# harvard-edge/multilingual_kws

Hardware: AMD Instinct MI355X
Metric: clips/sec end-to-end (log-mel + embedding fwd), batch 1024, 1s@16kHz (higher is better)
Workload: dtype f32; 1 GPU; configs[2]: batch=1024/GPU synthetic 1s@16kHz clips -> micro-frontend (int16 fixed-point, fp32 I/O) -> EfficientNet-B0 embedding forward (frozen, fp32 MFMA pointwise conv) -> [1024,1024]; clips_per_gpu=1024, samples_per_clip=16000, weights=synthetic seed 1234, parallelism=clip-sharded x1, build=47cee32cb12851f8

## Files before the change

multilingual_kws_amd/csrc/mkws_embed.hip:

```cpp
#include "mkws_common.h"
#include "mkws_embed_arch.h"

#include <algorithm>
#include <cmath>
#include <cstdlib>
#include <map>
#include <mutex>
#include <new>
#include <set>
#include <string>
#include <type_traits>
#include <vector>

#pragma clang fp contract(fast)
#include "mkws_embed_dev.h"
#include "mkws_embed_rows.h"

namespace mkws {

__device__ __forceinline__ int opaque_(int v) { asm volatile("" : "+v"(v)); return v; }
__device__ __forceinline__ float apply_act(float v, int act) {
  switch (act) {
    case ACT_SWISH: return swishf_(v);
    case ACT_RELU: return v > 0.0f ? v : 0.0f;
// ... 1014 lines not shown
  static constexpr int MTI = (G * HW + 15) / 16, MTO = (G * HoWo + 15) / 16;
  static constexpr int NW4 = KCT * NTC * 64, NS1 = NW4 + 2 * Q, NS2 = KS * KS * Q + 2 * Q;
  static constexpr int oX = 0;
  static constexpr int oS1 = oX + KCT * MTI * 256;
  static constexpr int oS2 = oS1 + NS1 * 4;
  static constexpr int oE = oS2 + NS2 * 4;
  static constexpr int oD = oE + (G * HW + 1) * LDE;
  static constexpr int oMean = oD + G * HoWo * LDD;
  static constexpr int oGate = oMean + G * CEXP;
  static constexpr int oR = oGate + G * CEXP;
  static constexpr int lds_floats = oR + G * 16;
  static_assert(NSEG * SEG == WoT, "segments tile the output row");
  static_assert(CEXP % CC == 0 && CC % 16 == 0, "chunks are whole MFMA tiles");
};

template <int KS, int S, int KCT, int HT, int WT, int CEXP, int CC, int NTP, int G, int SEG, int NTHR, int WPE, bool PAIR = false>
__global__ __launch_bounds__(NTHR, WPE) void mbconv_mid_kernel(MidArgs a) {
  using GM = MidGeom<KS, S, KCT, HT, WT, CEXP, CC, G, SEG>;
  constexpr int HW = GM::HW, HoT = GM::HoT, WoT = GM::WoT, HoWo = GM::HoWo, PT = GM::PT, PLF = GM::PLF;
  constexpr int NSEG = GM::NSEG, NC = GM::NC, Q = GM::Q, NTC = GM::NTC, LDE = GM::LDE, LDD = GM::LDD, NCH = GM::NCH, KC = GM::KC;
  constexpr int MTI = GM::MTI, MTO = GM::MTO, NW4 = GM::NW4, NS1 = GM::NS1, NS2 = GM::NS2;
  constexpr int NW = NTHR / 64;
  constexpr int SE_MAX = 10;
  constexpr int TAP_ROW_UNROLL = (KS == 5) ? 1 : KS;
  constexpr int NSL = NTHR / 16;
  constexpr int CPS = (CEXP + NSL - 1) / NSL;
  constexpr int CQ = CEXP / 4;
  constexpr int RS = NTHR / (G * CQ);
  constexpr int R1 = (NS1 + NTHR - 1) / NTHR, R2 = (NS2 + NTHR - 1) / NTHR;
  static_assert(NTHR % 64 == 0 && NTHR >= CEXP && NTHR >= 16 * G && RS >= 1, "thread roles");
  static_assert(NTHR * G <= KCT * MTI * 256 && G * RS * CEXP <= GM::oD - GM::oS1, "aliased scratch fits");
  extern __shared__ __attribute__((aligned(16))) float s_mid[];
  MKWS_WG_BEGIN();
  float* s_X = s_mid + GM::oX;
  float* s_part = s_X;
  float* s_W = s_mid + GM::oS1;
  float* s_scE = s_W + NW4 * 4;
  float* s_wd = s_mid + GM::oS2;
  float* s_scD = s_wd + KS * KS * CC;
  float* s_E = s_mid + GM::oE;
  f32x4* s_csum = reinterpret_cast<f32x4*>(s_W);
  float* s_D = s_mid + GM::oD;
  float* s_mean = s_mid + GM::oMean;
  float* s_gate = s_mid + GM::oGate;
  float* s_r = s_mid + GM::oR;
  const int tid = threadIdx.x, lane = tid & 63;
  const int wave = __builtin_amdgcn_readfirstlane(tid >> 6);
  const int g = lane >> 4, c = lane & 15;
  const int b0 = blockIdx.x * G;
  const int gvalid = (a.B - b0 < G) ? (a.B - b0) : G;
  const int rows = gvalid * HW, rows_out = gvalid * HoWo;
  const size_t row0_in = (size_t)b0 * HW, row0_out = (size_t)b0 * HoWo;
#ifdef MKWS_FRONT_TIMING
  unsigned long long* dbgp = a.dbg_t + (size_t)blockIdx.x * 8;
  unsigned long long t_p1 = 0, t_p2 = 0, t_red = 0, t_mark = 0;
  if (tid == 0) { t_mark = wall_clock64(); dbgp[0] = t_mark; }
#endif
  auto src1 = [&](int e, int chn) -> const float* {
    if (e < NW4) {
      const int l = e & 63, jn = e >> 6, j = jn / NTC, ntl = jn - j * NTC;
      return a.WpE + (((size_t)j * a.NTtotE + chn * NTC + ntl) * 64 + l) * 4;
    }
    const int q = e - NW4;
    return (q < Q ? a.scE + 4 * q : a.shE + 4 * (q - Q)) + chn * CC;
  };
  auto src2 = [&](int e, int chn) -> const float* {
    if (e < KS * KS * Q) {
      const int t = e / Q, q = e - t * Q;
      return a.Wd + (size_t)t * CEXP + chn * CC + 4 * q;
    }
    const int q = e - KS * KS * Q;
// ... 161 lines not shown
      }
    }
    if (chn + 1 < NCH) store1();
    __syncthreads();
#ifdef MKWS_FRONT_TIMING
    if (tid == 0) { const unsigned long long t = wall_clock64(); t_p2 += t - t_mark; t_mark = t; }
#endif
  }
  if (MKWS_ABLATE(16)) request_se();
  constexpr int NWP = NW / NTP;
  constexpr int MTW = (MTO + NWP - 1) / NWP;
  constexpr int PD = (KC >= 8) ? 8 : 4;
  const int ntp = wave % NTP, rlp = wave / NTP;
  const WBuf p_w(a.WpP, (unsigned)(g * 64 + c * 4));
  f32x4 wqp[PD][1];
  if (rlp < NWP) stream_mfma_prefetch<1, PD>(wqp, p_w, (size_t)NTP * 256, ntp, 1, NTP, KC);
  if (a.dbg_dw) {
    for (int i = tid; i < rows_out * CQ; i += NTHR) {
      const int r = i / CQ, q4 = (i - r * CQ) * 4;
      *reinterpret_cast<f32x4*>(a.dbg_dw + (row0_out + r) * CEXP + q4) = *reinterpret_cast<const f32x4*>(s_D + (size_t)r * LDD + q4);
    }
  }
  if (!MKWS_ABLATE(4)) {
  if (tid < G * RS * CQ) {
    const int q = tid % CQ, rs = (tid / CQ) % RS, gi = tid / (CQ * RS);
    f32x4 t = {0.f, 0.f, 0.f, 0.f};
    for (int r = rs; r < HoWo; r += RS) t += *reinterpret_cast<const f32x4*>(s_D + (size_t)(gi * HoWo + r) * LDD + 4 * q);
    s_csum[tid] = t;
  }
  __syncthreads();
  if (tid < G * CQ) {
    const int q = tid % CQ, gi = tid / CQ;
    f32x4 t = s_csum[(size_t)gi * RS * CQ + q];
#pragma unroll 4
    for (int rs = 1; rs < RS; ++rs) t += s_csum[((size_t)gi * RS + rs) * CQ + q];
    *reinterpret_cast<f32x4*>(s_mean + (size_t)gi * CEXP + 4 * q) = t * (1.0f / (float)HoWo);
  }
  __syncthreads();
  {
    const int n = tid & 15, sl = tid >> 4;
#pragma unroll
    for (int gi = 0; gi < G; ++gi) {
      float v = 0.0f;
// ... 18 lines not shown
#pragma unroll
    for (int gi = 0; gi < G; ++gi) {
      float v = be_pre;
#pragma unroll
      for (int n2 = 0; n2 < SE_MAX; ++n2) v += s_r[gi * 16 + n2] * we_pre[n2];
      const float gt = sigmoidf_(v);
      s_gate[gi * CEXP + tid] = gt;
      if (a.dbg_gate && gi < gvalid) a.dbg_gate[(size_t)(b0 + gi) * CEXP + tid] = gt;
    }
  }
  __syncthreads();
  }
#ifdef MKWS_FRONT_TIMING
  if (tid == 0) { const unsigned long long t = wall_clock64(); t_red += t - t_mark; t_mark = t; }
#endif
  if (rlp < NWP && !MKWS_ABLATE(8)) {
    constexpr int MT_LO = MTO / NWP;
    const int my_tiles = (MTO - rlp + NWP - 1) / NWP;
    auto run = [&](auto mt_tag) {
      constexpr int MT = decltype(mt_tag)::value;
      const float* erow[MT];
      const float* grow[MT];
#pragma unroll
      for (int m = 0; m < MT; ++m) {
        int r = (rlp + NWP * m) * 16 + c;
        if (r >= G * HoWo) r = G * HoWo - 1;
        erow[m] = s_D + (size_t)r * LDD + 4 * g;
        grow[m] = s_gate + (size_t)(r / HoWo) * CEXP + 4 * g;
      }
      struct EG { f32x4 e, g; };
      auto xload = [&](int j, int m) { return EG{*reinterpret_cast<const f32x4*>(erow[m] + 16 * j), *reinterpret_cast<const f32x4*>(grow[m] + 16 * j)}; };
// ... 13 lines not shown
            if (a.residual) y += *reinterpret_cast<const f32x4*>(a.X + (row0_in + r) * a.Cin + n);
            *reinterpret_cast<f32x4*>(a.Y + (row0_out + r) * a.Cout + n) = y;
          }
        }
      }
    };
    if constexpr (MT_LO >= 1 && MT_LO < MTW) {
      if (my_tiles >= MTW) run(std::integral_constant<int, MTW>{});
      else run(std::integral_constant<int, MT_LO>{});
    } else {
      run(std::integral_constant<int, MTW>{});
    }
  }
#ifdef MKWS_FRONT_TIMING
  __syncthreads();
  if (tid == 0) { const unsigned long long t = wall_clock64(); dbgp[1] = t_p1; dbgp[2] = t_p2; dbgp[3] = t_red; dbgp[4] = t - t_mark; dbgp[5] = t; }
#endif
  MKWS_WG_END();
}

struct BackArgs {
  const float* D; const float* X; int Cin;
  const float* Wr; const float* br; const float* We; const float* be; int se;
  const float* WpP; const float* scP; const float* shP;
  float* Y; int Cout; int residual;
  float* dbg_gate;
  int B;
};

template <int HOWO, int CEXP, int NTP, int RS, int NTHR, int WPE>
__global__ __launch_bounds__(NTHR, WPE) void mbconv_back_kernel(BackArgs a) {
  constexpr int LDD = CEXP + 4, CQ = CEXP / 4, KC = CEXP / 16, MTO = (HOWO + 15) / 16, NW = NTHR / 64;
// ... 655 lines not shown
#ifdef MKWS_FRONT_TIMING
  __syncthreads();
  if (threadIdx.x == 0) { a.dbg_t[(size_t)blockIdx.x * 8 + 6] = wall_clock64(); a.dbg_t[(size_t)blockIdx.x * 8 + 7] = (unsigned long long)(clock64() - dbg_c0); }
#endif
}

constexpr int kChainMax = 6;
struct ChainArgs {
  const BlockArgs* tab;
  int i0, n;
  unsigned kinds;
  const float* X; float* Y;
  int B;
  int ldsU, ldsE;
  int se4;
#ifdef MKWS_FRONT_TIMING
  unsigned long long* dbg_t;
#endif
};

__device__ __forceinline__ int sgpr_(int v) { return __builtin_amdgcn_readfirstlane(v); }
template <typename T>
__device__ __forceinline__ T* sgpr_(T* p) {
  const unsigned long long v = reinterpret_cast<unsigned long long>(p);
  const unsigned lo = (unsigned)__builtin_amdgcn_readfirstlane((int)(unsigned)v), hi = (unsigned)__builtin_amdgcn_readfirstlane((int)(unsigned)(v >> 32));
  typedef __attribute__((address_space(1))) T* gptr_t;
  return (T*)reinterpret_cast<gptr_t>(((unsigned long long)hi << 32) | lo);
}
__device__ __forceinline__ BlockArgs sgpr_block_args(const BlockArgs& t) {
  BlockArgs a;
// ... 355 lines not shown
template <int MT, int NWAVES>
__global__ __launch_bounds__(NWAVES * 64) void mbconv_chain_kernel(ChainArgs ca) {
  extern __shared__ __attribute__((aligned(16))) float s_blk[];
  constexpr int NTHR = NWAVES * 64;
  constexpr int HW = 12, G = MT * 16 / HW;
  const BlockArgs* __restrict__ tab = ca.tab + ca.i0;
  const int tid = threadIdx.x, lane = tid & 63;
  const int wave = __builtin_amdgcn_readfirstlane(tid >> 6);
  const int g = lane >> 4, c = lane & 15;
#ifdef MKWS_FRONT_TIMING
  if (ca.dbg_t && threadIdx.x == 0) ca.dbg_t[(size_t)gridDim.x * kChainMax * 8 + blockIdx.x] = wall_clock64();
#endif
  f32x4 carry[MT];
#pragma unroll
  for (int m = 0; m < MT; ++m) carry[m] = (f32x4){0.f, 0.f, 0.f, 0.f};
  {
    const int Cin = sgpr_(tab[0].Cin), KCe = sgpr_(tab[0].KCe), Cexp = sgpr_(tab[0].Cexp);
    const int b0 = blockIdx.x * G;
    const int gvalid = (ca.B - b0 < G) ? (ca.B - b0) : G;
    const int rows_in = gvalid * HW;
    const size_t row0_in = (size_t)b0 * HW;
    float* s_X = s_blk;
    float* s_scE = s_blk + ca.ldsU + ca.ldsE;
    for (int jm = wave; jm < KCe * MT; jm += NWAVES) {
      const int j = jm / MT, m = jm - j * MT;
      const int r = m * 16 + c;
      f32x4 v = {0.f, 0.f, 0.f, 0.f};
      if (r < rows_in && 16 * j + 4 * g < Cin) v = *reinterpret_cast<const f32x4*>(ca.X + (row0_in + r) * Cin + 16 * j + 4 * g);
      *reinterpret_cast<f32x4*>(s_X + ((size_t)jm * 64 + lane) * 4) = v;
    }
    const float* scE = sgpr_(tab[0].scE); const float* shE = sgpr_(tab[0].shE);
// ... 1 lines not shown
    __syncthreads();
  }
  for (int i = 0; i < ca.n; ++i) {
    BlockArgs a = sgpr_block_args(tab[i]);
    const bool last = (i + 1 == ca.n);
    if (!ca.se4) a.WrQ = nullptr;
    a.X = ca.X; a.Y = ca.Y; a.B = ca.B;
    const BlockArgs* nxp = last ? tab + i : tab + i + 1;
    const unsigned kind = (ca.kinds >> (2 * i)) & 3u;
#ifdef MKWS_FRONT_TIMING
    unsigned long long* dt = ca.dbg_t ? ca.dbg_t + ((size_t)blockIdx.x * kChainMax + i) * 8 : nullptr;
    if (dt && threadIdx.x == 0) dt[7] = wall_clock64();
#else
    unsigned long long* dt = nullptr;
#endif
    if (kind == 0) chain_block<3, 1, MT, NWAVES>(a, nxp, !last, s_blk, ca.ldsU, ca.ldsE, i == 0, carry, dt);
    else if (kind == 1) chain_block<5, 1, MT, NWAVES>(a, nxp, !last, s_blk, ca.ldsU, ca.ldsE, i == 0, carry, dt);
    else chain_block<5, 2, MT, NWAVES>(a, nxp, !last, s_blk, ca.ldsU, ca.ldsE, i == 0, carry, dt);
  }
}

#ifdef MKWS_PAIR_NT_STORES
#define MKWS_XSTORE(ptr, val) __builtin_nontemporal_store((val), (ptr))
#else
#define MKWS_XSTORE(ptr, val) (*(ptr) = (val))
#endif

struct PairArgs {
  BlockArgs b;
  float* xc1;
  float* xd;
  int* flags;
  int* err_dev;
// ... 1402 lines not shown
  float* se_part = nullptr;
  float* splitk_ws = nullptr; size_t splitk_floats = 0;
  const float *stem_w = nullptr, *stem_scale = nullptr, *stem_shift = nullptr;
  float norm_mean = 0.f, norm_std = 1.f;
  bool fuse_front = true;
  int fuse_gap = 1;
  int fuse_stem = 1;
  int fuse_back = 1;
  int fuse_mid = 1;
  int fuse_gemv = 1;
  int fuse_se4 = 1;
  int fuse_walk = 1;
  int fuse_rows = 0;
  int fuse_block = 2;
  int fuse_chain = 1;
  mkws::BlockArgs* d_chain_tab = nullptr;
  int fuse_top = 1;
  int fuse_pair = 1;
  float* pair_xc1 = nullptr; float* pair_xd = nullptr; int* pair_flags = nullptr;
  int* pair_err_dev = nullptr;
  int* pair_err_host = nullptr;
  size_t pair_flag_count = 0;
  int* pair_chain_flags = nullptr;
  int pair_fault = 0;
  int pair_degraded = 0;
  int fuse_cluster = 0;
  float* cl_xc1 = nullptr; float* cl_xd = nullptr; int* cl_flags = nullptr; size_t cl_flag_count = 0;
  int fuse_cluster_chain = 0;
  int pair_mt = 2;
  int block_mt43 = 3;
// ... 478 lines not shown
}
static bool chain_link_ok(const BlockPlan& b, const BlockPlan& next) {
  if (b.spec.stride != 1) return false;
  if (b.project.NTtot > kBlockWaves) return false;
  if (next.spec.in_ch != b.spec.out_ch || next.expand.KC != b.project.NTtot) return false;
  return next.ce <= 3 * kBlockWaves * 64;
}
bool cluster_supported(const BlockPlan& b);
bool pair_supported(const BlockPlan& b);
static bool chain_member(const mkws_embed* em, const BlockPlan& b) {
  if (!(em->fuse_chain == 1 || em->fuse_chain == 2) || !em->fuse_block || !block_supported(b, em->fuse_block)) return false;
  if (!(b.H == 4 && b.W == 3)) return false;
  if (em->fuse_cluster && cluster_supported(b) && em->cl_flags) return false;
  return true;
}
int launch_chain(hipStream_t s, const mkws_embed* em, int i0, int i1, const float* X, float* Y, int B) {
  ChainArgs ca;
  const int n = i1 - i0 + 1, mt43 = em->block_mt43;
  if (!em->d_chain_tab) return fail(MKWS_ERR_UNSUPPORTED, "chain: no block table");
  ca.tab = em->d_chain_tab; ca.i0 = i0; ca.n = n; ca.kinds = 0; ca.ldsU = ca.ldsE = 0;
  ca.X = X; ca.Y = Y; ca.B = B; ca.se4 = em->fuse_se4;
  int ldsZ = 0;
  std::string names;
  for (int k = 0; k < n; ++k) {
    const BlockPlan& b = em->blocks[i0 + k];
    const int ks = b.spec.kernel, st = b.spec.stride;
    if (ks == 3 && st != 1) return fail(MKWS_ERR_UNSUPPORTED, "chain: 3x3 stride-2 block");
    ca.kinds |= (unsigned)((ks == 3 && st == 1) ? 0 : (ks == 5 && st == 1) ? 1 : 2) << (2 * k);
    const int MT = block_row_tiles(b, mt43), G = MT * 16 / (b.H * b.W);
    const BlockLds L = block_lds(b.expand.KC, b.ce, MT, G, kBlockWaves);
    ca.ldsU = std::max(ca.ldsU, L.U); ca.ldsE = std::max(ca.ldsE, L.E); ldsZ = std::max(ldsZ, L.Z);
    names += (k ? "," : "") + std::string(b.spec.name);
  }
  const size_t lds = ((size_t)ca.ldsU + ca.ldsE + ldsZ) * sizeof(float);
  if (lds > 160 * 1024) return fail(MKWS_ERR_UNSUPPORTED, "chain: LDS carve %zu bytes", lds);
  const int G = mt43 * 16 / 12;
  const dim3 grid((B + G - 1) / G);
  ProfScope ps("chain:" + names, std::string("mbconv_chain_kernel<") + std::to_string(mt43) + "," + std::to_string(kBlockWaves) + ">");
#ifdef MKWS_FRONT_TIMING
  static unsigned long long* d_ct = nullptr;
  const size_t nstamp = (size_t)grid.x * kChainMax * 8 + grid.x;
  if (!d_ct) (void)hipMalloc(&d_ct, sizeof(unsigned long long) * (4096 * kChainMax * 8 + 4096));
  ca.dbg_t = (grid.x <= 4096) ? d_ct : nullptr;
#endif
  if (mt43 == 3) {
    if (int rc_ = ensure_dynamic_lds(reinterpret_cast<const void*>(&mbconv_chain_kernel<3, kBlockWaves>), 160 * 1024)) return rc_;
    hipLaunchKernelGGL((mbconv_chain_kernel<3, kBlockWaves>), grid, dim3(kBlockWaves * 64), lds, s, ca);
  } else if (mt43 == 2) {
    if (int rc_ = ensure_dynamic_lds(reinterpret_cast<const void*>(&mbconv_chain_kernel<2, kBlockWaves>), 160 * 1024)) return rc_;
    hipLaunchKernelGGL((mbconv_chain_kernel<2, kBlockWaves>), grid, dim3(kBlockWaves * 64), lds, s, ca);
  } else {
    if (int rc_ = ensure_dynamic_lds(reinterpret_cast<const void*>(&mbconv_chain_kernel<1, kBlockWaves>), 160 * 1024)) return rc_;
    hipLaunchKernelGGL((mbconv_chain_kernel<1, kBlockWaves>), grid, dim3(kBlockWaves * 64), lds, s, ca);
  }
#ifdef MKWS_FRONT_TIMING
  if (ca.dbg_t) {
    (void)hipStreamSynchronize(s);
    std::vector<unsigned long long> h(nstamp);
    (void)hipMemcpy(h.data(), d_ct, nstamp * 8, hipMemcpyDeviceToHost);
    unsigned long long t0 = ~0ull, t1 = 0;
    for (unsigned w = 0; w < grid.x; ++w) {
      t0 = std::min(t0, h[(size_t)grid.x * kChainMax * 8 + w]);
      t1 = std::max(t1, h[((size_t)w * kChainMax + (n - 1)) * 8 + 6]);
    }
    double pro = 0;
    for (unsigned w = 0; w < grid.x; ++w) pro += (double)(h[((size_t)w * kChainMax) * 8 + 7] - h[(size_t)grid.x * kChainMax * 8 + w]);
    fprintf(stderr, "[chain-timing] %s: %u workgroups, span %.2f us, prologue %.2f us\n", names.c_str(), grid.x, (double)(t1 - t0) / 100.0, pro / grid.x / 100.0);
    for (int k = 0; k < n; ++k) {
      double ph[7] = {0, 0, 0, 0, 0, 0, 0};
      unsigned long long e_min = ~0ull, e_max = 0;
      for (unsigned w = 0; w < grid.x; ++w) {
        const unsigned long long* q = &h[((size_t)w * kChainMax + k) * 8];
        ph[0] += (double)(q[0] - q[7]);
        for (int j = 0; j < 6; ++j) ph[j + 1] += (double)(q[j + 1] - q[j]);
        e_min = std::min(e_min, q[6]); e_max = std::max(e_max, q[6]);
      }
      fprintf(stderr, "[chain-timing]   %s: args %.2f  A %.2f  B %.2f  C1 %.2f  C2 %.2f  gate %.2f  D %.2f us; end skew %.2f us\n", em->blocks[i0 + k].spec.name,
              ph[0] / grid.x / 100.0, ph[1] / grid.x / 100.0, ph[2] / grid.x / 100.0, ph[3] / grid.x / 100.0, ph[4] / grid.x / 100.0, ph[5] / grid.x / 100.0,
              ph[6] / grid.x / 100.0, (double)(e_max - e_min) / 100.0);
    }
  }
#endif
// ... 307 lines not shown
          stage, CC, G, grid.x, NTHR, lds, p1 / grid.x / 100.0, p2 / grid.x / 100.0, se / grid.x / 100.0, pj / grid.x / 100.0, tot / grid.x / 100.0, (double)(t1 - t0) / 100.0);
  MKWS_WG_TRACE_REPORT(s, stage, "mid", (size_t)grid.x);
#else
  hipLaunchKernelGGL(fn, grid, dim3(NTHR), lds, s, a);
#endif
  return MKWS_OK;
}

bool mid_enabled(const BlockPlan& b, int fuse_mid) {
  if (!fuse_mid || !mid_supported(b)) return false;
  if (fuse_mid == 2) return true;
  if (b.H == 13 && b.spec.kernel == 3) return fuse_mid == 1;
  return (b.H == 13 && b.spec.kernel == 5) || (b.H == 7 && b.spec.stride == 2);
}

int launch_mid(hipStream_t s, const char* stage, const BlockPlan& b, int one_clip, const float* X, float* Y, float* dbg_dw, float* dbg_gate, int B) {
  MidArgs a;
  a.X = X; a.Cin = b.spec.in_ch;
  a.WpE = b.expand.Wp; a.scE = b.expand.scale; a.shE = b.expand.shift; a.NTtotE = b.expand.NTtot;
  a.Wd = b.dw.Wd; a.scD = b.dw.scale; a.shD = b.dw.shift;
  a.Wr = b.se.Wr; a.br = b.se.br; a.We = b.se.We; a.be = b.se.be; a.se = b.se.se;
  a.WpP = b.project.Wp; a.scP = b.project.scale; a.shP = b.project.shift;
  a.Y = Y; a.Cout = b.spec.out_ch; a.residual = b.residual ? 1 : 0;
  a.dbg_dw = dbg_dw; a.dbg_gate = dbg_gate; a.B = B;
  const int ks = b.spec.kernel, st = b.spec.stride;
  if (b.H == 25) return launch_mid_inst<3, 2, 1, 25, 20, 96, 16, 2, 1, 1, 1024, 4>(s, stage, a);
  if (b.H == 13 && ks == 3) return launch_mid_inst<3, 1, 2, 13, 10, 144, 48, 2, 1, 5, 1024, 4, true>(s, stage, a);
  if (b.H == 13) return launch_mid_inst<5, 2, 2, 13, 10, 144, 48, 3, 1, 5, 512, 4, true>(s, stage, a);
  if (st == 1) return launch_mid_inst<5, 1, 3, 7, 5, 240, 48, 3, 1, 1, 512, 4>(s, stage, a);
  if (one_clip) return launch_mid_inst<3, 2, 3, 7, 5, 240, 48, 5, 1, 3, 512, 4, true>(s, stage, a);
  return launch_mid_inst<3, 2, 3, 7, 5, 240, 48, 5, 2, 3, 512, 4, true>(s, stage, a);
}

int rows_variant(const BlockPlan& b) {
  if (!b.has_expand || b.se.se > 10 || b.spec.stride != 1 || !b.residual) return -1;
  const int ks = b.spec.kernel, ci = b.spec.in_ch, co = b.spec.out_ch;
  if (b.H == 13 && b.W == 10 && ks == 3 && ci == 24 && co == 24 && b.ce == 144 && b.project.NTtot == 2) return kRows2b;
  if (b.H == 7 && b.W == 5 && ks == 5 && ci == 40 && co == 40 && b.ce == 240 && b.project.NTtot == 3) return kRows3b;
  return -1;
// ... 117 lines not shown
#ifdef MKWS_FRONT_TIMING
    wg_phase_report("block1a: prologue / stem / depthwise + next stage / SE / projection", (size_t)(B < device_cu_count() ? B : device_cu_count()), 5);
#endif
  } else {
    const long pix = (long)B * 500;
    int grid = (int)((pix + 31) / 32);
    if (grid > 8192) grid = 8192;
    ProfScope ps("stem", "stem_kernel");
    hipLaunchKernelGGL(stem_kernel, dim3(grid), dim3(256), 0, s, d_spec, em->stem_w, em->stem_scale, em->stem_shift,
                       em->norm_mean, em->norm_std, em->bufA, B);
    if (hit("stem", em->bufA, (size_t)B * 500 * kStemCh)) return MKWS_OK;
  }
  float* cur = em->bufA;
  float* nxt = em->bufB;
  bool top_done = false;
  for (int i = 0; i < kNumBlocks; ++i) {
    const BlockPlan& b = em->blocks[i];
    const std::string p = std::string("block") + b.spec.name;
    const int Min = B * b.H * b.W, Mout = B * b.Ho * b.Wo;
    if (i == 0 && fused_1a) {
      if (hit(p, nxt, (size_t)Mout * b.spec.out_ch)) return MKWS_OK;
      float* t = cur; cur = nxt; nxt = t;
      continue;
    }
    const bool want_expand_tap = stop && (p + "_expand") == stop;
    if (em->fuse_rows && rows_variant(b) >= 0 && !want_expand_tap) {
      const bool tap_dw = stop && (p + "_dw") == stop, tap_gate = stop && (p + "_gate") == stop;
      if (int rc = launch_rows(s, p.c_str(), b, em->fuse_rows == 2, cur, nxt, tap_dw ? em->bufD : nullptr, tap_gate ? em->gate : nullptr, B)) return rc;
      if (hit(p + "_dw", em->bufD, (size_t)Mout * b.ce)) return MKWS_OK;
      if (hit(p + "_gate", em->gate, (size_t)B * b.ce)) return MKWS_OK;
      if (hit(p, nxt, (size_t)Mout * b.spec.out_ch)) return MKWS_OK;
      float* t = cur; cur = nxt; nxt = t;
      continue;
    }
    if (mid_enabled(b, em->fuse_mid) && !want_expand_tap) {
      const bool tap_dw = stop && (p + "_dw") == stop, tap_gate = stop && (p + "_gate") == stop;
      if (int rc = launch_mid(s, p.c_str(), b, em->block_mt43 == 1, cur, nxt, tap_dw ? em->bufD : nullptr, tap_gate ? em->gate : nullptr, B)) return rc;
      if (hit(p + "_dw", em->bufD, (size_t)Mout * b.ce)) return MKWS_OK;
      if (hit(p + "_gate", em->gate, (size_t)B * b.ce)) return MKWS_OK;
      if (hit(p, nxt, (size_t)Mout * b.spec.out_ch)) return MKWS_OK;
      float* t = cur; cur = nxt; nxt = t;
      continue;
    }
    {
      auto inner_tap = [&](int j) {
        if (!stop) return false;
        const std::string q = std::string("block") + em->blocks[j].spec.name;
        return (q + "_expand") == stop || (q + "_dw") == stop || (q + "_gate") == stop;
      };
      if (chain_member(em, b) && !inner_tap(i)) {
        int e = i;
        while (e + 1 < kNumBlocks && e + 1 - i < kChainMax && !(stop && (std::string("block") + em->blocks[e].spec.name) == stop) &&
               chain_member(em, em->blocks[e + 1]) && chain_link_ok(em->blocks[e], em->blocks[e + 1]) && !inner_tap(e + 1)) ++e;
        const BlockPlan& bl = em->blocks[e];
        if (int rc = launch_chain(s, em, i, e, cur, nxt, B)) return rc;
        if (hit(std::string("block") + bl.spec.name, nxt, (size_t)B * bl.Ho * bl.Wo * bl.spec.out_ch)) return MKWS_OK;
        float* t = cur; cur = nxt; nxt = t;
        i = e;
        continue;
      }
      if (pair_chain_member(em, b) && !inner_tap(i)) {
        int e = i;
        while (e + 1 < kNumBlocks && e + 1 - i < kPairChainMax && !(stop && (std::string("block") + em->blocks[e].spec.name) == stop) &&
               pair_chain_member(em, em->blocks[e + 1]) && pair_chain_link_ok(em->blocks[e], em->blocks[e + 1]) && !inner_tap(e + 1)) ++e;
        const BlockPlan& bl = em->blocks[e];
        const bool with_top = em->fuse_top && em->fuse_gap && (!stop || strcmp(stop, "gap") == 0 || strncmp(stop, "dense", 5) == 0) && e == kNumBlocks - 1 && em->topH * em->topW == 4;
        if (int rc = launch_pair_chain(s, em, i, e, cur, nxt, B, with_top)) return rc;
        top_done = with_top;
        if (hit(std::string("block") + bl.spec.name, nxt, (size_t)B * bl.Ho * bl.Wo * bl.spec.out_ch)) return MKWS_OK;
        float* t = cur; cur = nxt; nxt = t;
        i = e;
        continue;
      }
    }
    if (B == 1 && em->fuse_block && em->fuse_cluster_chain && cluster_supported(b) && !stop) {
// ... 350 lines not shown
  return MKWS_OK;
}

int mkws_embed_set_option(mkws_embed* em, const char* name, int value) {
  if (!em || !name) return fail(MKWS_ERR_INVALID_ARG, "NULL argument");
  if (strcmp(name, "fuse_front") == 0) { em->fuse_front = value != 0; return MKWS_OK; }
  if (strcmp(name, "fuse_block") == 0) { em->fuse_block = value; return MKWS_OK; }
  if (strcmp(name, "fuse_mid") == 0) { em->fuse_mid = value; return MKWS_OK; }
  if (strcmp(name, "fuse_rows") == 0) { em->fuse_rows = value; return MKWS_OK; }
  if (strcmp(name, "fuse_walk") == 0) { em->fuse_walk = value; return MKWS_OK; }
  if (strcmp(name, "fuse_se4") == 0) { em->fuse_se4 = value ? 1 : 0; return MKWS_OK; }
  if (strcmp(name, "fuse_gemv") == 0) { em->fuse_gemv = value; return MKWS_OK; }
  if (strcmp(name, "fuse_back") == 0) { em->fuse_back = value; return MKWS_OK; }
  if (strcmp(name, "fuse_pair") == 0) { em->fuse_pair = value; return MKWS_OK; }
  if (strcmp(name, "fuse_chain") == 0) { em->fuse_chain = value; return MKWS_OK; }
  if (strcmp(name, "fuse_top") == 0) { em->fuse_top = value; return MKWS_OK; }
  if (strcmp(name, "fuse_cluster") == 0) {
    if (value && !em->cl_flags) return fail(MKWS_ERR_UNSUPPORTED, "fuse_cluster needs a handle of at most 64 clips (max_batch = %d)", em->max_batch);
    em->fuse_cluster = value; return MKWS_OK;
  }
  if (strcmp(name, "fuse_cluster_chain") == 0) {
    if (value && (em->max_batch != 1 || !em->cl_flags)) return fail(MKWS_ERR_UNSUPPORTED, "fuse_cluster_chain is the plan of one-clip handles (max_batch = %d)", em->max_batch);
    em->fuse_cluster_chain = value; return MKWS_OK;
  }
  if (strcmp(name, "fuse_stem") == 0) { em->fuse_stem = value; return MKWS_OK; }
  if (strcmp(name, "big_tiles") == 0) {
    if (value) { em->pair_mt = 2; em->block_mt43 = 3; } else { em->pair_mt = pair_row_tiles(em->plan_batch); em->block_mt43 = block43_row_tiles(em->plan_batch); }
    return MKWS_OK;
  }
  if (strcmp(name, "plan_batch") == 0) {
// ... 20 lines not shown
  return fail(MKWS_ERR_INVALID_ARG, "unknown option '%s'", name);
}

int mkws_embed_get_option(const mkws_embed* em, const char* name) {
  if (!em || !name) return fail(MKWS_ERR_INVALID_ARG, "NULL argument");
  if (strcmp(name, "fuse_front") == 0) return em->fuse_front ? 1 : 0;
  if (strcmp(name, "fuse_block") == 0) return em->fuse_block;
  if (strcmp(name, "fuse_mid") == 0) return em->fuse_mid;
  if (strcmp(name, "fuse_rows") == 0) return em->fuse_rows;
  if (strcmp(name, "fuse_walk") == 0) return em->fuse_walk;
  if (strcmp(name, "fuse_se4") == 0) return em->fuse_se4;
  if (strcmp(name, "fuse_gemv") == 0) return em->fuse_gemv;
  if (strcmp(name, "fuse_back") == 0) return em->fuse_back;
  if (strcmp(name, "fuse_pair") == 0) return em->fuse_pair;
  if (strcmp(name, "fuse_chain") == 0) return em->fuse_chain;
  if (strcmp(name, "fuse_top") == 0) return em->fuse_top;
  if (strcmp(name, "fuse_cluster") == 0) return em->fuse_cluster;
  if (strcmp(name, "fuse_cluster_chain") == 0) return em->fuse_cluster_chain;
  if (strcmp(name, "fuse_stem") == 0) return em->fuse_stem;
  if (strcmp(name, "fuse_gap") == 0) return em->fuse_gap;
  if (strcmp(name, "block_tiles") == 0) return em->block_mt43;
  if (strcmp(name, "pair_degraded") == 0) return em->pair_degraded;
  if (strcmp(name, "guard_floats") == 0) return (int)em->guard;
  if (strcmp(name, "guard_bands") == 0) return (int)em->guard_spans.size();
  if (strcmp(name, "guard_violations") == 0) return guard_violations(em);
  if (strcmp(name, "exchange_error") == 0) return em->pair_err_host ? *reinterpret_cast<volatile int*>(em->pair_err_host) : 0;
  if (strcmp(name, "max_batch") == 0) return em->max_batch;
  if (strcmp(name, "plan_batch") == 0) return em->plan_batch;
  return fail(MKWS_ERR_INVALID_ARG, "unknown option '%s'", name);
}
// ... 50 lines not shown
```

Baseline: 1.092 million clips/s.

## Fuse block 4a mid kernel into the following chain kernel as a prologue

Refactors the mid kernel body into a device function and calls it as a prologue inside the chain kernel for block 4a (stride-2, 240 expand). The projected output stays in LDS as MFMA fragments and is handed to the first chain block as its carry, so the 4a output never goes through global memory and one kernel launch is dropped. A new wave dealing gives the last row tile's projection to the extra waves. The cost is that the chain kernel now needs the larger LDS carve of the two stages, which may lower occupancy, and the scale and shift loads have to be staged around the prologue.

```diff
diff --git a/multilingual_kws_amd/csrc/mkws_embed.hip b/multilingual_kws_amd/csrc/mkws_embed.hip
--- a/multilingual_kws_amd/csrc/mkws_embed.hip
+++ b/multilingual_kws_amd/csrc/mkws_embed.hip
@@ -1052,8 +1052,8 @@
   static_assert(CEXP % CC == 0 && CC % 16 == 0, "chunks are whole MFMA tiles");
 };
 
-template <int KS, int S, int KCT, int HT, int WT, int CEXP, int CC, int NTP, int G, int SEG, int NTHR, int WPE, bool PAIR = false>
-__global__ __launch_bounds__(NTHR, WPE) void mbconv_mid_kernel(MidArgs a) {
+template <int KS, int S, int KCT, int HT, int WT, int CEXP, int CC, int NTP, int G, int SEG, int NTHR, bool PAIR, int RSF, bool LINK>
+__device__ __forceinline__ void mid_body(const MidArgs& a, float* s_mid) {
   using GM = MidGeom<KS, S, KCT, HT, WT, CEXP, CC, G, SEG>;
   constexpr int HW = GM::HW, HoT = GM::HoT, WoT = GM::WoT, HoWo = GM::HoWo, PT = GM::PT, PLF = GM::PLF;
   constexpr int NSEG = GM::NSEG, NC = GM::NC, Q = GM::Q, NTC = GM::NTC, LDE = GM::LDE, LDD = GM::LDD, NCH = GM::NCH, KC = GM::KC;
@@ -1064,12 +1064,10 @@
   constexpr int NSL = NTHR / 16;
   constexpr int CPS = (CEXP + NSL - 1) / NSL;
   constexpr int CQ = CEXP / 4;
-  constexpr int RS = NTHR / (G * CQ);
+  constexpr int RS = RSF ? RSF : NTHR / (G * CQ);
   constexpr int R1 = (NS1 + NTHR - 1) / NTHR, R2 = (NS2 + NTHR - 1) / NTHR;
-  static_assert(NTHR % 64 == 0 && NTHR >= CEXP && NTHR >= 16 * G && RS >= 1, "thread roles");
+  static_assert(NTHR % 64 == 0 && NTHR >= CEXP && NTHR >= 16 * G && NTHR >= G * CQ && RS >= 1, "thread roles");
   static_assert(NTHR * G <= KCT * MTI * 256 && G * RS * CEXP <= GM::oD - GM::oS1, "aliased scratch fits");
-  extern __shared__ __attribute__((aligned(16))) float s_mid[];
-  MKWS_WG_BEGIN();
   float* s_X = s_mid + GM::oX;
   float* s_part = s_X;
   float* s_W = s_mid + GM::oS1;
@@ -1090,9 +1088,9 @@
   const int rows = gvalid * HW, rows_out = gvalid * HoWo;
   const size_t row0_in = (size_t)b0 * HW, row0_out = (size_t)b0 * HoWo;
 #ifdef MKWS_FRONT_TIMING
-  unsigned long long* dbgp = a.dbg_t + (size_t)blockIdx.x * 8;
+  unsigned long long* dbgp = a.dbg_t ? a.dbg_t + (size_t)blockIdx.x * 8 : nullptr;
   unsigned long long t_p1 = 0, t_p2 = 0, t_red = 0, t_mark = 0;
-  if (tid == 0) { t_mark = wall_clock64(); dbgp[0] = t_mark; }
+  if (tid == 0 && dbgp) { t_mark = wall_clock64(); dbgp[0] = t_mark; }
 #endif
   auto src1 = [&](int e, int chn) -> const float* {
     if (e < NW4) {
@@ -1284,7 +1282,14 @@
   const int ntp = wave % NTP, rlp = wave / NTP;
   const WBuf p_w(a.WpP, (unsigned)(g * 64 + c * 4));
   f32x4 wqp[PD][1];
-  if (rlp < NWP) stream_mfma_prefetch<1, PD>(wqp, p_w, (size_t)NTP * 256, ntp, 1, NTP, KC);
+  const bool lrow = LINK && wave >= NTP;
+  const int lt0 = 2 * (wave - NTP);
+  f32x4 wql[PD][2];
+  if (LINK) {
+    static_assert(!LINK || (MTO >= 2 && MTO * 16 == G * HoWo && NTP <= 2 * (NW - NTP) && NTP <= NW), "link dealing");
+    if (!lrow) stream_mfma_prefetch<1, PD>(wqp, p_w, (size_t)NTP * 256, wave, 1, NTP, KC);
+    else stream_mfma_prefetch<2, PD>(wql, p_w, (size_t)NTP * 256, lt0, 1, NTP, KC);
+  } else if (rlp < NWP) stream_mfma_prefetch<1, PD>(wqp, p_w, (size_t)NTP * 256, ntp, 1, NTP, KC);
   if (a.dbg_dw) {
     for (int i = tid; i < rows_out * CQ; i += NTHR) {
       const int r = i / CQ, q4 = (i - r * CQ) * 4;
@@ -1292,11 +1297,11 @@
     }
   }
   if (!MKWS_ABLATE(4)) {
-  if (tid < G * RS * CQ) {
-    const int q = tid % CQ, rs = (tid / CQ) % RS, gi = tid / (CQ * RS);
+  for (int it = tid; it < G * RS * CQ; it += NTHR) {
+    const int q = it % CQ, rs = (it / CQ) % RS, gi = it / (CQ * RS);
     f32x4 t = {0.f, 0.f, 0.f, 0.f};
     for (int r = rs; r < HoWo; r += RS) t += *reinterpret_cast<const f32x4*>(s_D + (size_t)(gi * HoWo + r) * LDD + 4 * q);
-    s_csum[tid] = t;
+    s_csum[it] = t;
   }
   __syncthreads();
   if (tid < G * CQ) {
@@ -1345,7 +1350,49 @@
 #ifdef MKWS_FRONT_TIMING
   if (tid == 0) { const unsigned long long t = wall_clock64(); t_red += t - t_mark; t_mark = t; }
 #endif
-  if (rlp < NWP && !MKWS_ABLATE(8)) {
+  if constexpr (LINK) {
+   if (!MKWS_ABLATE(8)) {
+    struct EG { f32x4 e, g; };
+    auto xmake = [](const EG& v) { return v.e * v.g; };
+    auto rows_of = [&](int rt, const float*& er, const float*& gr) {
+      const int r = rt * 16 + c;
+      er = s_D + (size_t)r * LDD + 4 * g;
+      gr = s_gate + (size_t)(r / HoWo) * CEXP + 4 * g;
+    };
+    auto fin = [&](const f32x4& acc, int t, int rt) {
+      const int n = t * 16 + 4 * g, r = rt * 16 + c;
+      f32x4 y = {0.f, 0.f, 0.f, 0.f};
+      if (r < rows_out) {
+        y = acc * *reinterpret_cast<const f32x4*>(a.scP + n) + *reinterpret_cast<const f32x4*>(a.shP + n);
+        if (a.residual) y += *reinterpret_cast<const f32x4*>(a.X + (row0_in + r) * a.Cin + n);
+      }
+      *reinterpret_cast<f32x4*>(s_mid + ((size_t)(t * MTO + rt) * 64 + lane) * 4) = y;
+    };
+    if (!lrow) {
+      constexpr int MT = MTO - 1;
+      const float* erow[MT];
+      const float* grow[MT];
+#pragma unroll
+      for (int m = 0; m < MT; ++m) rows_of(m, erow[m], grow[m]);
+      auto xload = [&](int j, int m) { return EG{*reinterpret_cast<const f32x4*>(erow[m] + 16 * j), *reinterpret_cast<const f32x4*>(grow[m] + 16 * j)}; };
+      f32x4 acc[1][MT];
+#pragma unroll
+      for (int m = 0; m < MT; ++m) acc[0][m] = (f32x4){0.f, 0.f, 0.f, 0.f};
+      stream_mfma<1, PD, MT, true>(acc, wqp, p_w, (size_t)NTP * 256, wave, 1, NTP, KC, xload, xmake);
+#pragma unroll
+      for (int m = 0; m < MT; ++m) fin(acc[0][m], wave, m);
+    } else {
+      const float* er; const float* gr;
+      rows_of(MTO - 1, er, gr);
+      auto xload = [&](int j, int) { return EG{*reinterpret_cast<const f32x4*>(er + 16 * j), *reinterpret_cast<const f32x4*>(gr + 16 * j)}; };
+      f32x4 acc[2][1] = {{{0.f, 0.f, 0.f, 0.f}}, {{0.f, 0.f, 0.f, 0.f}}};
+      stream_mfma<2, PD, 1, true>(acc, wql, p_w, (size_t)NTP * 256, lt0, 1, NTP, KC, xload, xmake);
+#pragma unroll
+      for (int q = 0; q < 2; ++q)
+        if (lt0 + q < NTP) fin(acc[q][0], lt0 + q, MTO - 1);
+    }
+   }
+  } else if (rlp < NWP && !MKWS_ABLATE(8)) {
     constexpr int MT_LO = MTO / NWP;
     const int my_tiles = (MTO - rlp + NWP - 1) / NWP;
     auto run = [&](auto mt_tag) {
@@ -1389,8 +1436,15 @@
   }
 #ifdef MKWS_FRONT_TIMING
   __syncthreads();
-  if (tid == 0) { const unsigned long long t = wall_clock64(); dbgp[1] = t_p1; dbgp[2] = t_p2; dbgp[3] = t_red; dbgp[4] = t - t_mark; dbgp[5] = t; }
-#endif
+  if (tid == 0 && dbgp) { const unsigned long long t = wall_clock64(); dbgp[1] = t_p1; dbgp[2] = t_p2; dbgp[3] = t_red; dbgp[4] = t - t_mark; dbgp[5] = t; }
+#endif
+}
+
+template <int KS, int S, int KCT, int HT, int WT, int CEXP, int CC, int NTP, int G, int SEG, int NTHR, int WPE, bool PAIR = false>
+__global__ __launch_bounds__(NTHR, WPE) void mbconv_mid_kernel(MidArgs a) {
+  extern __shared__ __attribute__((aligned(16))) float s_mid[];
+  MKWS_WG_BEGIN();
+  mid_body<KS, S, KCT, HT, WT, CEXP, CC, NTP, G, SEG, NTHR, PAIR, 0, false>(a, s_mid);
   MKWS_WG_END();
 }
 
@@ -2076,6 +2130,8 @@
   int B;
   int ldsU, ldsE;
   int se4;
+  int link4a;
+  MidArgs a4;
 #ifdef MKWS_FRONT_TIMING
   unsigned long long* dbg_t;
 #endif
@@ -2461,7 +2517,45 @@
   f32x4 carry[MT];
 #pragma unroll
   for (int m = 0; m < MT; ++m) carry[m] = (f32x4){0.f, 0.f, 0.f, 0.f};
-  {
+  bool link = false;
+  if constexpr (MT == 3) link = ca.link4a != 0;
+  if constexpr (MT == 3) {
+    if (link) {
+      constexpr int NCST = 3;
+      const int Cexp = sgpr_(tab[0].Cexp);
+      float nsc[NCST], nsh[NCST];
+      {
+        const float* scE = sgpr_(tab[0].scE); const float* shE = sgpr_(tab[0].shE);
+#pragma unroll
+        for (int k = 0; k < NCST; ++k) {
+          const int i = tid + k * NTHR;
+          if (i < Cexp) { nsc[k] = scE[i]; nsh[k] = shE[i]; }
+        }
+      }
+      mid_body<3, 2, 3, 7, 5, 240, 48, 5, 4, 3, NTHR, true, 4, true>(ca.a4, s_blk);
+      __syncthreads();
+      const int NTp = sgpr_(tab[0].NTp);
+      const bool rowsplit = (NTp == NWAVES / 2 + 1) && (MT <= NWAVES / 2 - 1);
+      auto frag = [&](int t, int m) { return *reinterpret_cast<const f32x4*>(s_blk + ((size_t)(t * MT + m) * 64 + lane) * 4); };
+      if (rowsplit) {
+        if (wave < NWAVES / 2) {
+#pragma unroll
+          for (int m = 0; m < MT; ++m) carry[m] = frag(wave, m);
+        } else if (wave < NWAVES / 2 + MT) carry[0] = frag(NTp - 1, wave - NWAVES / 2);
+      } else if (wave < NTp) {
+#pragma unroll
+        for (int m = 0; m < MT; ++m) carry[m] = frag(wave, m);
+      }
+      float* s_scE = s_blk + ca.ldsU + ca.ldsE;
+#pragma unroll
+      for (int k = 0; k < NCST; ++k) {
+        const int i = tid + k * NTHR;
+        if (i < Cexp) { s_scE[i] = nsc[k]; s_scE[Cexp + i] = nsh[k]; }
+      }
+      __syncthreads();
+    }
+  }
+  if (!link) {
     const int Cin = sgpr_(tab[0].Cin), KCe = sgpr_(tab[0].KCe), Cexp = sgpr_(tab[0].Cexp);
     const int b0 = blockIdx.x * G;
     const int gvalid = (ca.B - b0 < G) ? (ca.B - b0) : G;
@@ -2493,9 +2587,10 @@
 #else
     unsigned long long* dt = nullptr;
 #endif
-    if (kind == 0) chain_block<3, 1, MT, NWAVES>(a, nxp, !last, s_blk, ca.ldsU, ca.ldsE, i == 0, carry, dt);
-    else if (kind == 1) chain_block<5, 1, MT, NWAVES>(a, nxp, !last, s_blk, ca.ldsU, ca.ldsE, i == 0, carry, dt);
-    else chain_block<5, 2, MT, NWAVES>(a, nxp, !last, s_blk, ca.ldsU, ca.ldsE, i == 0, carry, dt);
+    const bool first = i == 0 && !link;
+    if (kind == 0) chain_block<3, 1, MT, NWAVES>(a, nxp, !last, s_blk, ca.ldsU, ca.ldsE, first, carry, dt);
+    else if (kind == 1) chain_block<5, 1, MT, NWAVES>(a, nxp, !last, s_blk, ca.ldsU, ca.ldsE, first, carry, dt);
+    else chain_block<5, 2, MT, NWAVES>(a, nxp, !last, s_blk, ca.ldsU, ca.ldsE, first, carry, dt);
   }
 }
 
@@ -3928,6 +4023,7 @@
   int fuse_rows = 0;
   int fuse_block = 2;
   int fuse_chain = 1;
+  int fuse_chain_4a = 1;
   mkws::BlockArgs* d_chain_tab = nullptr;
   int fuse_top = 1;
   int fuse_pair = 1;
@@ -4436,14 +4532,29 @@
   if (em->fuse_cluster && cluster_supported(b) && em->cl_flags) return false;
   return true;
 }
-int launch_chain(hipStream_t s, const mkws_embed* em, int i0, int i1, const float* X, float* Y, int B) {
+using Link4aGeom = MidGeom<3, 2, 3, 7, 5, 240, 48, 4, 3>;
+void fill_mid_args(MidArgs& a, const BlockPlan& b, const float* X, float* Y, float* dbg_dw, float* dbg_gate, int B);
+bool mid_enabled(const BlockPlan& b, int fuse_mid);
+static bool chain_link4a_ok(const mkws_embed* em, const BlockPlan& b, const BlockPlan& first) {
+  return em->fuse_chain_4a && em->block_mt43 == 3 && mid_enabled(b, em->fuse_mid) && b.H == 7 && b.W == 5 && b.spec.stride == 2 && b.spec.kernel == 3 &&
+         b.ce == 240 && b.spec.in_ch == 40 && b.spec.out_ch == 80 && b.project.NTtot == 5 && first.spec.stride == 1 && first.spec.in_ch == 80 &&
+         first.expand.KC == 5 && first.ce <= 3 * kBlockWaves * 64 && (size_t)Link4aGeom::lds_floats * sizeof(float) <= 160 * 1024;
+}
+int launch_chain(hipStream_t s, const mkws_embed* em, int i0, int i1, const float* X, float* Y, int B, const BlockPlan* link4a = nullptr) {
   ChainArgs ca;
   const int n = i1 - i0 + 1, mt43 = em->block_mt43;
   if (!em->d_chain_tab) return fail(MKWS_ERR_UNSUPPORTED, "chain: no block table");
   ca.tab = em->d_chain_tab; ca.i0 = i0; ca.n = n; ca.kinds = 0; ca.ldsU = ca.ldsE = 0;
   ca.X = X; ca.Y = Y; ca.B = B; ca.se4 = em->fuse_se4;
+  ca.link4a = 0; ca.a4 = MidArgs{};
   int ldsZ = 0;
   std::string names;
+  if (link4a) {
+    if (mt43 != 3 || !chain_link4a_ok(em, *link4a, em->blocks[i0])) return fail(MKWS_ERR_UNSUPPORTED, "chain: 4a link on this plan");
+    ca.link4a = 1;
+    fill_mid_args(ca.a4, *link4a, X, nullptr, nullptr, nullptr, B);
+    names = std::string(link4a->spec.name) + ",";
+  }
   for (int k = 0; k < n; ++k) {
     const BlockPlan& b = em->blocks[i0 + k];
     const int ks = b.spec.kernel, st = b.spec.stride;
@@ -4454,7 +4565,8 @@
     ca.ldsU = std::max(ca.ldsU, L.U); ca.ldsE = std::max(ca.ldsE, L.E); ldsZ = std::max(ldsZ, L.Z);
     names += (k ? "," : "") + std::string(b.spec.name);
   }
-  const size_t lds = ((size_t)ca.ldsU + ca.ldsE + ldsZ) * sizeof(float);
+  size_t lds = ((size_t)ca.ldsU + ca.ldsE + ldsZ) * sizeof(float);
+  if (link4a) lds = std::max(lds, (size_t)Link4aGeom::lds_floats * sizeof(float));
   if (lds > 160 * 1024) return fail(MKWS_ERR_UNSUPPORTED, "chain: LDS carve %zu bytes", lds);
   const int G = mt43 * 16 / 12;
   const dim3 grid((B + G - 1) / G);
@@ -4464,6 +4576,9 @@
   const size_t nstamp = (size_t)grid.x * kChainMax * 8 + grid.x;
   if (!d_ct) (void)hipMalloc(&d_ct, sizeof(unsigned long long) * (4096 * kChainMax * 8 + 4096));
   ca.dbg_t = (grid.x <= 4096) ? d_ct : nullptr;
+  static unsigned long long* d_lt = nullptr;
+  if (!d_lt) (void)hipMalloc(&d_lt, sizeof(unsigned long long) * 8 * 4096);
+  if (ca.link4a && grid.x <= 4096) ca.a4.dbg_t = d_lt;
 #endif
   if (mt43 == 3) {
     if (int rc_ = ensure_dynamic_lds(reinterpret_cast<const void*>(&mbconv_chain_kernel<3, kBlockWaves>), 160 * 1024)) return rc_;
@@ -4488,6 +4603,14 @@
     double pro = 0;
     for (unsigned w = 0; w < grid.x; ++w) pro += (double)(h[((size_t)w * kChainMax) * 8 + 7] - h[(size_t)grid.x * kChainMax * 8 + w]);
     fprintf(stderr, "[chain-timing] %s: %u workgroups, span %.2f us, prologue %.2f us\n", names.c_str(), grid.x, (double)(t1 - t0) / 100.0, pro / grid.x / 100.0);
+    if (ca.a4.dbg_t) {
+      std::vector<unsigned long long> l((size_t)grid.x * 8);
+      (void)hipMemcpy(l.data(), d_lt, l.size() * 8, hipMemcpyDeviceToHost);
+      double p1 = 0, p2 = 0, se = 0, pj = 0;
+      for (unsigned w = 0; w < grid.x; ++w) { p1 += (double)l[8 * w + 1]; p2 += (double)l[8 * w + 2]; se += (double)l[8 * w + 3]; pj += (double)l[8 * w + 4]; }
+      fprintf(stderr, "[chain-timing]   4a link: expand %.2f  depthwise %.2f  SE %.2f  project %.2f us per workgroup (the rest of the prologue: hand-over to the first block)\n",
+              p1 / grid.x / 100.0, p2 / grid.x / 100.0, se / grid.x / 100.0, pj / grid.x / 100.0);
+    }
     for (int k = 0; k < n; ++k) {
       double ph[7] = {0, 0, 0, 0, 0, 0, 0};
       unsigned long long e_min = ~0ull, e_max = 0;
@@ -4825,8 +4948,7 @@
   return (b.H == 13 && b.spec.kernel == 5) || (b.H == 7 && b.spec.stride == 2);
 }
 
-int launch_mid(hipStream_t s, const char* stage, const BlockPlan& b, int one_clip, const float* X, float* Y, float* dbg_dw, float* dbg_gate, int B) {
-  MidArgs a;
+void fill_mid_args(MidArgs& a, const BlockPlan& b, const float* X, float* Y, float* dbg_dw, float* dbg_gate, int B) {
   a.X = X; a.Cin = b.spec.in_ch;
   a.WpE = b.expand.Wp; a.scE = b.expand.scale; a.shE = b.expand.shift; a.NTtotE = b.expand.NTtot;
   a.Wd = b.dw.Wd; a.scD = b.dw.scale; a.shD = b.dw.shift;
@@ -4834,6 +4956,14 @@
   a.WpP = b.project.Wp; a.scP = b.project.scale; a.shP = b.project.shift;
   a.Y = Y; a.Cout = b.spec.out_ch; a.residual = b.residual ? 1 : 0;
   a.dbg_dw = dbg_dw; a.dbg_gate = dbg_gate; a.B = B;
+#ifdef MKWS_FRONT_TIMING
+  a.dbg_t = nullptr;
+#endif
+}
+
+int launch_mid(hipStream_t s, const char* stage, const BlockPlan& b, int one_clip, const float* X, float* Y, float* dbg_dw, float* dbg_gate, int B) {
+  MidArgs a;
+  fill_mid_args(a, b, X, Y, dbg_dw, dbg_gate, B);
   const int ks = b.spec.kernel, st = b.spec.stride;
   if (b.H == 25) return launch_mid_inst<3, 2, 1, 25, 20, 96, 16, 2, 1, 1, 1024, 4>(s, stage, a);
   if (b.H == 13 && ks == 3) return launch_mid_inst<3, 1, 2, 13, 10, 144, 48, 2, 1, 5, 1024, 4, true>(s, stage, a);
@@ -4981,6 +5111,7 @@
   float* cur = em->bufA;
   float* nxt = em->bufB;
   bool top_done = false;
+  const BlockPlan* link4a = nullptr;
   for (int i = 0; i < kNumBlocks; ++i) {
     const BlockPlan& b = em->blocks[i];
     const std::string p = std::string("block") + b.spec.name;
@@ -5001,6 +5132,14 @@
       continue;
     }
     if (mid_enabled(b, em->fuse_mid) && !want_expand_tap) {
+      if (i + 1 < kNumBlocks && !(stop && strncmp(stop, p.c_str(), p.size()) == 0) && chain_link4a_ok(em, b, em->blocks[i + 1]) &&
+          chain_member(em, em->blocks[i + 1])) {
+        const std::string q = std::string("block") + em->blocks[i + 1].spec.name;
+        if (!stop || !((q + "_expand") == stop || (q + "_dw") == stop || (q + "_gate") == stop)) {
+          link4a = &b;
+          continue;
+        }
+      }
       const bool tap_dw = stop && (p + "_dw") == stop, tap_gate = stop && (p + "_gate") == stop;
       if (int rc = launch_mid(s, p.c_str(), b, em->block_mt43 == 1, cur, nxt, tap_dw ? em->bufD : nullptr, tap_gate ? em->gate : nullptr, B)) return rc;
       if (hit(p + "_dw", em->bufD, (size_t)Mout * b.ce)) return MKWS_OK;
@@ -5020,12 +5159,14 @@
         while (e + 1 < kNumBlocks && e + 1 - i < kChainMax && !(stop && (std::string("block") + em->blocks[e].spec.name) == stop) &&
                chain_member(em, em->blocks[e + 1]) && chain_link_ok(em->blocks[e], em->blocks[e + 1]) && !inner_tap(e + 1)) ++e;
         const BlockPlan& bl = em->blocks[e];
-        if (int rc = launch_chain(s, em, i, e, cur, nxt, B)) return rc;
+        if (int rc = launch_chain(s, em, i, e, cur, nxt, B, link4a)) return rc;
+        link4a = nullptr;
         if (hit(std::string("block") + bl.spec.name, nxt, (size_t)B * bl.Ho * bl.Wo * bl.spec.out_ch)) return MKWS_OK;
         float* t = cur; cur = nxt; nxt = t;
         i = e;
         continue;
       }
+      if (link4a) return fail(MKWS_ERR_UNSUPPORTED, "block %s: no chain to take the 4a link", b.spec.name);
       if (pair_chain_member(em, b) && !inner_tap(i)) {
         int e = i;
         while (e + 1 < kNumBlocks && e + 1 - i < kPairChainMax && !(stop && (std::string("block") + em->blocks[e].spec.name) == stop) &&
@@ -5406,6 +5547,7 @@
   if (strcmp(name, "fuse_back") == 0) { em->fuse_back = value; return MKWS_OK; }
   if (strcmp(name, "fuse_pair") == 0) { em->fuse_pair = value; return MKWS_OK; }
   if (strcmp(name, "fuse_chain") == 0) { em->fuse_chain = value; return MKWS_OK; }
+  if (strcmp(name, "fuse_chain_4a") == 0) { em->fuse_chain_4a = value ? 1 : 0; return MKWS_OK; }
   if (strcmp(name, "fuse_top") == 0) { em->fuse_top = value; return MKWS_OK; }
   if (strcmp(name, "fuse_cluster") == 0) {
     if (value && !em->cl_flags) return fail(MKWS_ERR_UNSUPPORTED, "fuse_cluster needs a handle of at most 64 clips (max_batch = %d)", em->max_batch);
@@ -5456,6 +5598,7 @@
   if (strcmp(name, "fuse_back") == 0) return em->fuse_back;
   if (strcmp(name, "fuse_pair") == 0) return em->fuse_pair;
   if (strcmp(name, "fuse_chain") == 0) return em->fuse_chain;
+  if (strcmp(name, "fuse_chain_4a") == 0) return em->fuse_chain_4a;
   if (strcmp(name, "fuse_top") == 0) return em->fuse_top;
   if (strcmp(name, "fuse_cluster") == 0) return em->fuse_cluster;
   if (strcmp(name, "fuse_cluster_chain") == 0) return em->fuse_cluster_chain;
```

Result: faster. 1.107 million clips/s, median of 6 (+1.4%).
